# EnyaHermite/SPH3D-GCN

Hardware: AMD Instinct MI355X
Metric: point-cloud blocks/sec (fwd+bwd) SPH3D_s3dis 8192-pt (higher is better)
Workload: dtype f32

## Files before the change

### include/sph3d.h

```cpp
#ifndef SPH3D_H
#define SPH3D_H

#include <stddef.h>

#ifdef __cplusplus
extern "C" {
#endif

typedef void* sph3d_stream_t;

enum {
    SPH3D_OK = 0,
    SPH3D_EINVAL = -1,
    SPH3D_EWORKSPACE = -2,
    SPH3D_ELAUNCH = -3,
    SPH3D_EUNSUPPORTED = -4
};

#define SPH3D_ABI_VERSION 2
int sph3d_abi_version(void);
const char* sph3d_last_error(void);
const char* sph3d_build_info(void);


// ... 67 lines not shown
                                const int* nn_index, const int* nn_count, const int* bin_index,
                                const float* input, const float* filter, const float* grad_output,
                                float* grad_input, float* grad_filter,
                                void* workspace, size_t workspace_bytes,
                                sph3d_stream_t stream);

size_t sph3d_graph_transpose_workspace(int B, int N, int M, int K, int F);
int sph3d_graph_transpose(int B, int N, int M, int K, int F,
                          const int* nn_index, const int* nn_count,
                          const int* bin_index , const float* weight ,
                          int* offsets, int* ent_key, float* ent_scale,
                          int* active_bins ,
                          void* workspace, size_t workspace_bytes, sph3d_stream_t stream);
int sph3d_graph_transpose_count(int B, int N, int M, int K, int F, const int* nn_index, const int* nn_count,
                                const int* bin_index, int want_active, void* workspace, size_t workspace_bytes,
                                sph3d_stream_t stream);
int sph3d_graph_transpose_finish(int B, int N, int M, int K, int F,
                                 const int* nn_index, const int* nn_count, const int* bin_index,
                                 const float* weight, int* offsets, int* ent_key, float* ent_scale, int* active_bins,
                                 void* workspace, size_t workspace_bytes, sph3d_stream_t stream);
int sph3d_gather_rows_count(int B, int N, int S, int K, const int* pairs, const int* nn_index, const int* nn_count,
                            int* out_index, int* out_count, void* transpose_workspace, size_t transpose_workspace_bytes,
                            sph3d_stream_t stream);
int sph3d_graph_transpose_finish_ordered(int B, int N, int M, int K, int F,
                                         const int* nn_index, const int* nn_count, const int* bin_index,
                                         const float* weight, int* offsets, int* ent_key, float* ent_scale, int* active_bins,
                                         int* order, void* workspace, size_t workspace_bytes, sph3d_stream_t stream);
int sph3d_graph_balanced_order(int B, int N, int F, const int* offsets, int* order, sph3d_stream_t stream);
int sph3d_set_deterministic(int on);
int sph3d_get_deterministic(void);
size_t sph3d_graph_canonical_order_workspace(int B, int N, int M, int K, int F);
int sph3d_graph_canonical_order(int B, int N, int M, int K, int F, const int* offsets, int* ent_key, float* ent_scale ,
                                void* workspace, size_t workspace_bytes, sph3d_stream_t stream);
size_t sph3d_depthwise_conv3d_grad_t_workspace(int B, int N, int F, int C, int r);
int sph3d_depthwise_conv3d_grad_t(int B, int N, int M, int F, int C, int r,
                                  const int* offsets, const int* ent_key, const float* ent_scale,
                                  const int* source_order ,
                                  const int* active_bins ,
                                  const float* input, const float* filter, const float* grad_output,
                                  float* grad_input, float* grad_filter,
                                  void* workspace, size_t workspace_bytes, sph3d_stream_t stream);

int sph3d_fuzzy_spherical_kernel(int B, int N, int M, int K, int n, int p, int q, float radius,
                                 const float* database, const float* query,
                                 const int* nn_index, const int* nn_count, const float* nn_dist,
                                 int* filt_index, int* filt_frac, sph3d_stream_t stream);
// ... 6 lines not shown
                                      const int* offsets, const int* ent_edge,
                                      const float* input, const float* filter, const float* grad_output,
                                      float* grad_input, float* grad_filter,
                                      void* workspace, size_t workspace_bytes, sph3d_stream_t stream);
int sph3d_graph_transpose_finish_edges(int B, int N, int M, int K, const int* nn_index, const int* nn_count,
                                       int* offsets, int* ent_edge, void* workspace, size_t workspace_bytes,
                                       sph3d_stream_t stream);

int sph3d_scatter_grad_t(int B, int Nin, int Mout, int C,
                         const int* offsets, const int* ent_key, const float* ent_scale,
                         const float* grad_output, float* grad_input, sph3d_stream_t stream);
size_t sph3d_scatter_grad_workspace(int B, int N, int M, int K);

int sph3d_max_pool3d(int B, int N, int M, int C, int K,
                     const int* nn_index, const int* nn_count, const float* input,
                     float* output, int* max_index, sph3d_stream_t stream);
int sph3d_max_pool3d_grad(int B, int N, int M, int C,
                          const int* max_index, const float* grad_output,
                          float* grad_input, sph3d_stream_t stream);
int sph3d_max_pool3d_grad_t(int B, int N, int M, int C, const int* offsets, const int* ent_key, const int* nn_count,
                            const int* max_index, const float* grad_output,
                            const float* addend ,
                            float* grad_input, sph3d_stream_t stream);
int sph3d_avg_pool3d(int B, int N, int M, int C, int K,
                     const int* nn_index, const int* nn_count, const float* input,
                     float* output, sph3d_stream_t stream);
int sph3d_avg_pool3d_grad(int B, int N, int M, int C, int K,
                          const int* nn_index, const int* nn_count, const float* grad_output,
                          float* grad_input,
                          void* workspace , size_t workspace_bytes,
                          sph3d_stream_t stream);

int sph3d_mean_interpolate(int B, int N, int M, int C, int K,
                           const int* nn_index, const int* nn_count, const float* input,
                           float* output, sph3d_stream_t stream);
int sph3d_mean_interpolate_grad(int B, int N, int M, int C, int K,
                                const int* nn_index, const int* nn_count, const float* grad_output,
                                float* grad_input,
                                void* workspace , size_t workspace_bytes,
                                sph3d_stream_t stream);
int sph3d_weighted_interpolate(int B, int N, int M, int C, int K,
                               const int* nn_index, const int* nn_count,
                               const float* input, const float* weight,
                               float* output, sph3d_stream_t stream);
int sph3d_weighted_interpolate_grad(int B, int N, int M, int C, int K,
                                    const int* nn_index, const int* nn_count,
// ... 273 lines not shown
```

### sph3d_gcn_amd/_lib.py

```python
import ctypes
import os

import torch

_HERE = os.path.dirname(os.path.abspath(__file__))
LIB_PATH = os.environ.get("SPH3D_LIB") or os.path.join(_HERE, "csrc", "libsph3d.so")

_c_int = ctypes.c_int
_c_float = ctypes.c_float
_c_size_t = ctypes.c_size_t
_vp = ctypes.c_void_p

_I, _F, _P, _S, _L = _c_int, _c_float, _vp, _c_size_t, ctypes.c_longlong


class AugmentParams(ctypes.Structure):
    _fields_ = [("threshold", ctypes.c_ulonglong * 9), ("enable", ctypes.c_uint), ("rgb_offset", _I), ("normal_offset", _I),
                ("max_nodes", _I), ("rgb_lo", _F), ("rgb_hi", _F), ("inv_g", _F * 2), ("scale", _F * 2)]


SIGNATURES = {
    "sph3d_abi_version": (_I, []),
    "sph3d_last_error": (ctypes.c_char_p, []),
    "sph3d_build_info": (ctypes.c_char_p, []),
# ... 4 lines not shown
    "sph3d_build_sphere_neighbor_ws": (_I, [_I, _I, _I, _I, _F, _P, _P, _P, _P, _P, _P, _S, _P]),
    "sph3d_build_sphere_neighbor_fixed_ws": (_I, [_I, _I, _I, _I, _F, _P, _P, _P, _P, _P, _P, _S, _P]),
    "sph3d_release_stream_scratch": (_I, [_P]),
    "sph3d_release_all_scratch": (_I, []),
    "sph3d_build_sphere_graph_ws": (_I, [_I, _I, _I, _I, _F, _I, _I, _I, _I] + [_P] * 6 + [_P, _S, _P, _S, _P]),
    "sph3d_build_cube_neighbor": (_I, [_I, _I, _I, _I, _I, _F, _P, _P, _P, _P, _P]),
    "sph3d_spherical_kernel": (_I, [_I, _I, _I, _I, _I, _I, _I, _F, _P, _P, _P, _P, _P, _P, _P]),
    "sph3d_spherical_kernel_ocml": (_I, [_I, _I, _I, _I, _I, _I, _I, _F, _P, _P, _P, _P, _P, _P, _P]),
    "sph3d_depthwise_conv3d": (_I, [_I] * 7 + [_P] * 7),
    "sph3d_depthwise_conv3d_grad_workspace": (_S, [_I] * 7),
    "sph3d_depthwise_conv3d_grad": (_I, [_I] * 7 + [_P] * 8 + [_P, _S, _P]),
    "sph3d_max_pool3d": (_I, [_I] * 5 + [_P] * 6),
    "sph3d_max_pool3d_grad": (_I, [_I] * 4 + [_P] * 4),
    "sph3d_max_pool3d_grad_t": (_I, [_I] * 4 + [_P] * 8),
    "sph3d_avg_pool3d": (_I, [_I] * 5 + [_P] * 5),
    "sph3d_avg_pool3d_grad": (_I, [_I] * 5 + [_P] * 4 + [_P, _S, _P]),
    "sph3d_graph_balanced_order": (_I, [_I, _I, _I, _P, _P, _P]),
    "sph3d_set_deterministic": (_I, [_I]),
    "sph3d_get_deterministic": (_I, []),
    "sph3d_graph_canonical_order_workspace": (_S, [_I] * 5),
    "sph3d_graph_canonical_order": (_I, [_I] * 5 + [_P] * 3 + [_P, _S, _P]),
    "sph3d_gather_nd": (_I, [_I, _I, ctypes.c_longlong, _I, _P, _P, _P, _P]),
    "sph3d_gather_rows_count": (_I, [_I] * 4 + [_P] * 5 + [_P, _S, _P]),
    "sph3d_graph_transpose_workspace": (_S, [_I] * 5),
    "sph3d_graph_transpose": (_I, [_I] * 5 + [_P] * 8 + [_P, _S, _P]),
    "sph3d_graph_transpose_count": (_I, [_I] * 5 + [_P] * 3 + [_I, _P, _S, _P]),
    "sph3d_graph_transpose_finish": (_I, [_I] * 5 + [_P] * 8 + [_P, _S, _P]),
    "sph3d_graph_transpose_finish_ordered": (_I, [_I] * 5 + [_P] * 9 + [_P, _S, _P]),
    "sph3d_build_sphere_graph": (_I, [_I, _I, _I, _I, _F, _I, _I, _I] + [_P] * 6 + [_P, _S, _P]),
    "sph3d_build_sphere_graph_ocml": (_I, [_I, _I, _I, _I, _F, _I, _I, _I] + [_P] * 6 + [_P, _S, _P]),
    "sph3d_depthwise_conv3d_grad_t_workspace": (_S, [_I] * 5),
    "sph3d_depthwise_conv3d_grad_t": (_I, [_I] * 6 + [_P] * 10 + [_P, _S, _P]),
    "sph3d_fuzzy_spherical_kernel": (_I, [_I, _I, _I, _I, _I, _I, _I, _F] + [_P] * 7 + [_P]),
    "sph3d_fuzzy_depthwise_conv3d": (_I, [_I] * 10 + [_P] * 7 + [_P]),
    "sph3d_fuzzy_depthwise_conv3d_grad_workspace": (_S, [_I] * 7),
    "sph3d_fuzzy_depthwise_conv3d_grad": (_I, [_I] * 10 + [_P] * 11 + [_P, _S, _P]),
    "sph3d_graph_transpose_finish_edges": (_I, [_I] * 4 + [_P] * 4 + [_P, _S, _P]),
    "sph3d_depthwise_conv3d_cat_supported": (_I, [_I] * 4),
    "sph3d_depthwise_conv3d_cat": (_I, [_I] * 8 + [_P] * 8),
    "sph3d_depthwise_conv3d_grad_t_cat": (_I, [_I] * 7 + [_P] * 12 + [_P, _S, _P]),
    "sph3d_depthwise_conv3d_plan": (_I, [_I] * 11 + [_P]),
    "sph3d_spatial_order": (_I, [_I, _I, _P, _P, _P]),
    "sph3d_scatter_grad_t": (_I, [_I] * 4 + [_P] * 6),
    "sph3d_scatter_grad_workspace": (_S, [_I] * 4),
    "sph3d_mean_interpolate": (_I, [_I] * 5 + [_P] * 5),
    "sph3d_mean_interpolate_grad": (_I, [_I] * 5 + [_P] * 4 + [_P, _S, _P]),
# ... 121 lines not shown
            fn.restype = res
            fn.argtypes = args
    if l.sph3d_abi_version() != ABI_VERSION:
        raise Sph3dError("libsph3d.so ABI version %d, this package binds version %d" % (l.sph3d_abi_version(), ABI_VERSION))
    _lib = _Proxy(l)
    return _lib


_timing = None


def timing_start():
    global _timing
    _timing = []


def timing_stop():
    global _timing
    out, _timing = _timing, None
    return out


_PURE = ("_workspace", "_blocks", "_supported", "_parts", "_sample_chunk")
_NO_TIME = ("sph3d_abi_version", "sph3d_last_error", "sph3d_build_info", "workspace", "_release_", "_blocks", "_supported", "_launches", "_parts", "_failures", "_mode", "_pieces", "_sample_chunk", "_plan")


class _Proxy:

    def __init__(self, cdll):
        self._cdll = cdll
        self._cache = {}
        self._memos = []

    def __getattr__(self, name):
        fn = getattr(self._cdll, name)
        if name == "sph3d_set_deterministic":
            def switch(on, _fn=fn, _memos=self._memos):
                prev = _fn(on)
                if (prev != 0) != (on != 0):
                    for m in _memos:
                        m.clear()
                return prev
            self.__dict__[name] = switch
            return switch
        if any(k in name for k in _PURE) and name != "sph3d_pointwise_gemm_bnstats_blocks":
            memo = {}
            self._memos.append(memo)
# ... 154 lines not shown
```

### sph3d_gcn_amd/_tgraph.py

```python
import collections
import contextlib

import torch

from . import _lib

BALANCE_MIN_POINTS = 1024
PACK_ENTRIES = True
_MAX_ENTRIES = 24
_cache = collections.OrderedDict()


def _ident(t):
    return (0, 0) if t is None else (t.data_ptr(), t._version)


_generation = [0]


def clear():
    _lib.release_scratch()
    _cache.clear()
    _orders.clear()
    _unique.clear()
# ... 31 lines not shown


def source_order(nn_index):
    hit = _orders.get(_ident(nn_index))
    if hit is None:
        return None
    order = hit[0]
    if order.is_cuda:
        cur = _lib.current_raw_stream()
        if cur not in hit[2]:
            order.record_stream(torch.cuda.current_stream())
            hit[2].add(cur)
    return order


_unique = set()


def peek(nn_index, nn_count, n_src, need_unique_rows=False):
    key = (_ident(nn_index), _ident(nn_count), _ident(None), _ident(None), int(n_src), 1, tuple(nn_index.shape))
    if key not in _cache or (need_unique_rows and key not in _unique):
        return None
    return transpose(nn_index, nn_count, n_src)


def _attach(nn_index, fkey, hit, nn_count, bin_index, weight):
    fast = nn_index.__dict__.get("_sph3d_tg")
    if fast is None:
        fast = nn_index._sph3d_tg = {}
    out, _keep, ev, synced = hit
    fast[fkey] = ((out, (nn_count, bin_index, weight), ev, synced),
                  (_generation[0], nn_index._version, nn_count._version, 0 if bin_index is None else bin_index._version,
                   0 if weight is None else weight._version))


def entries(tg):
    _off, key, scale, _act = tg
    if scale is not None:
        return key, scale
    cnt = (key >> 24) & 0xff
    return key & 0xffffff, torch.where(cnt > 0, 1.0 / cnt.float().clamp(min=1.0), torch.zeros_like(cnt, dtype=torch.float32))


def transpose(nn_index, nn_count, n_src, bin_index=None, weight=None, num_bins=1, counted_workspace=None, unique_rows=False):
    F = int(num_bins) if bin_index is not None else 1
    cur_raw = _lib.current_raw_stream()
# ... 102 lines not shown
```

### sph3d_gcn_amd/csrc/common.hpp

```cpp
#pragma once
#include <hip/hip_runtime.h>
#include <stdint.h>
#include <stdio.h>
#include <stdlib.h>
#include "../../include/sph3d.h"

namespace sph3d {

constexpr int kWave = 64;
constexpr int kRefGrid = 32;
constexpr int kRefBlock = 1024;

void set_error(const char* fmt, ...);

#define SPH3D_REQUIRE(cond, ...)                    \
    do {                                            \
        if (!(cond)) {                              \
            ::sph3d::set_error(__VA_ARGS__);        \
            return SPH3D_EINVAL;                    \
        }                                           \
    } while (0)

static inline int check_launch(const char* what)
{
// ... 68 lines not shown
static inline TgLayout tg_layout(void* workspace, int B, int N, int M, int K, int F)
{
    size_t off = 0;
    auto take = [&](size_t bytes) {
        char* p = workspace ? (char*)workspace + off : nullptr;
        off += (bytes + 255) & ~(size_t)255;
        return p;
    };
    TgLayout t;
    t.offsets = (int*)take(sizeof(int) * (size_t)B * ((size_t)N * F + 1));
    t.key = (int*)take(sizeof(int) * (size_t)B * M * K);
    t.scale = (float*)take(sizeof(float) * (size_t)B * M * K);
    t.active = (int*)take(sizeof(int) * ((size_t)F + 1));
    const size_t scratch_off = off;
    t.scratch = take(sph3d_graph_transpose_workspace(B, N, M, K, F));
    t.scratch_bytes = off - scratch_off;
    t.bytes = off;
    return t;
}

constexpr unsigned kTgKeyMask = 0x00ffffffu;
static inline bool tg_packable(int M, int K, const void* weight) { return weight == nullptr && M <= (1 << 24) && K <= 255; }

constexpr int kVoteMaxClasses = 64;
static inline int vote_check_args(const char* what, int B, int C, int num_blocks, long long total_rows, long long row_base,
                                  long long batch_rows)
{
    SPH3D_REQUIRE(B > 0 && B <= 65535, "%s: batch 0<B<=65535 required, got %d", what, B);
    SPH3D_REQUIRE(C > 0 && C <= kVoteMaxClasses, "%s: 0<C<=%d classes required, got %d", what, kVoteMaxClasses, C);
    SPH3D_REQUIRE(num_blocks > 0 && total_rows > 0, "%s: empty pool (num_blocks=%d total_rows=%lld)", what, num_blocks, total_rows);
    SPH3D_REQUIRE(row_base >= 0 && batch_rows > 0 && batch_rows <= 0x7fffffffll && row_base + batch_rows <= total_rows,
                  "%s: rows [%lld, %lld + %lld) are not a range of the pool's %lld", what, row_base, row_base, batch_rows, total_rows);
    return SPH3D_OK;
}

__device__ __forceinline__ int lane_id() { return (int)(threadIdx.x & 63); }

__device__ __forceinline__ int tg_key(int word, bool packed) { return packed ? (int)((unsigned)word & kTgKeyMask) : word; }
__device__ __forceinline__ float tg_packed_scale(int word) { return 1.0f / (float)((unsigned)word >> 24); }

__device__ __forceinline__ int prefix_popc(unsigned long long mask)
{
    return (int)__builtin_amdgcn_mbcnt_hi((unsigned)(mask >> 32), __builtin_amdgcn_mbcnt_lo((unsigned)mask, 0u));
}

__device__ __forceinline__ float elu1(float y) { return y > 0.f ? y : __expf(y) - 1.f; }
// ... 70 lines not shown
```

### sph3d_gcn_amd/csrc/graph.hip

```cpp
#include "common.hpp"

namespace sph3d {

__global__ __launch_bounds__(256) void zero_fill_kernel(unsigned* __restrict__ p, size_t words)
{
    const size_t head = ((16 - (reinterpret_cast<size_t>(p) & 15)) & 15) >> 2;
    const size_t h = head < words ? head : words;
    uint4* q = reinterpret_cast<uint4*>(p + h);
    const size_t quads = (words - h) >> 2;
    const size_t stride = (size_t)gridDim.x * blockDim.x;
    const size_t t = (size_t)blockIdx.x * blockDim.x + threadIdx.x;
    for (size_t i = t; i < quads; i += stride) q[i] = make_uint4(0u, 0u, 0u, 0u);
    if (t < h) p[t] = 0u;
    const size_t tail0 = h + (quads << 2);
    if (t < words - tail0) p[tail0 + t] = 0u;
}

int zero_async(void* p, size_t bytes, hipStream_t stream, const char* what)
{
    if (bytes == 0) return SPH3D_OK;
    if (bytes < (256u << 10) || (bytes & 3) != 0 || (reinterpret_cast<size_t>(p) & 3) != 0)
        return check_hip(hipMemsetAsync(p, 0, bytes, stream), what);
    const size_t words = bytes >> 2;
    size_t blocks = (words / 4 + 255) / 256;
// ... 685 lines not shown
                                       sph3d_stream_t stream)
{
    SPH3D_REQUIRE(B > 0 && N > 0 && S >= 0 && K > 0, "gather_rows_count: bad dims B=%d N=%d S=%d K=%d", B, N, S, K);
    if (S == 0) return SPH3D_OK;
    hipStream_t st = as_stream(stream);
    int* deg = nullptr;
    int* slot = nullptr;
    if (transpose_workspace != nullptr) {
        int rc = tg_dims_ok(B, N, S, K, 1, nullptr, transpose_workspace, transpose_workspace_bytes);
        if (rc) return rc;
        const TgWs w = tg_ws(transpose_workspace, B, N, S, K, 1);
        rc = zero_async(w.deg, sizeof(int) * w.zero_words, st, "gather_rows_count: memset");
        if (rc) return rc;
        deg = w.deg;
        slot = w.slot_pos;
    }
    long long blocks = ((long long)B * S + 3) / 4;
    if (blocks > 16384) blocks = 16384;
    hipLaunchKernelGGL(gather_rows_count_kernel, dim3((unsigned)blocks), dim3(256), 0, st, B, N, S, K, pairs, nn_index, nn_count, out_index,
                       out_count, deg, slot);
    return check_launch("sph3d_gather_rows_count");
}

extern "C" int sph3d_graph_transpose(int B, int N, int M, int K, int F,
                                     const int* nn_index, const int* nn_count, const int* bin_index,
                                     const float* weight, int* offsets, int* ent_key, float* ent_scale, int* active_bins,
                                     void* workspace, size_t workspace_bytes, sph3d_stream_t stream)
{
    int rc = sph3d_graph_transpose_count(B, N, M, K, F, nn_index, nn_count, bin_index, active_bins != nullptr, workspace,
                                         workspace_bytes, stream);
    if (rc) return rc;
    return sph3d_graph_transpose_finish(B, N, M, K, F, nn_index, nn_count, bin_index, weight, offsets, ent_key, ent_scale,
                                        active_bins, workspace, workspace_bytes, stream);
}
```

### sph3d_gcn_amd/csrc/pool3d.hip

```cpp
#include "common.hpp"

namespace sph3d {

constexpr int kPtsPerWG = 16;

enum class Mode { Max, Avg, Weighted };

template <Mode MODE, int V>
__global__ __launch_bounds__(256) void gather_fwd(
    int B, int Nin, int Mout, int C, int K, int mblocks,
    const int* __restrict__ nnIndex, const int* __restrict__ nnCount,
    const float* __restrict__ input, const float* __restrict__ weight,
    float* __restrict__ output, int* __restrict__ maxIndex, int ppwg)
{
    int b, mb;
    xcd_decode((int)blockIdx.x, B, mblocks, b, mb);
    if (b < 0) return;
    const int wave = uniform((int)threadIdx.x >> 6);
    const int lane = lane_id();
    const int m_begin = mb * ppwg;
    const int m_end = (m_begin + ppwg) < Mout ? (m_begin + ppwg) : Mout;
    const float* inb = input + (size_t)b * Nin * C;

    for (int m = m_begin + wave; m < m_end; m += 4) {
// ... 214 lines not shown
    for (int n = n_begin + wave; n < n_end; n += 4) {
        const int e0 = offb[n], e1 = offb[n + 1];
        for (int c0 = 0; c0 < C; c0 += 64 * V) {
            const int c = c0 + lane * V;
            const bool act = c < C;
            const int cc = act ? c : 0;
            float acc[V];
#pragma unroll
            for (int v = 0; v < V; v++) acc[v] = addend != nullptr ? addend[((size_t)b * Nin + n) * C + cc + v] : 0.f;
            auto take = [&](int m) {
                if (V == 4) {
                    const int4 a = *reinterpret_cast<const int4*>(&mib[(size_t)m * C + cc]);
                    const float4 g = *reinterpret_cast<const float4*>(&gob[(size_t)m * C + cc]);
                    acc[0] += a.x == n ? g.x : 0.f;
                    acc[1 % V] += a.y == n ? g.y : 0.f;
                    acc[2 % V] += a.z == n ? g.z : 0.f;
                    acc[3 % V] += a.w == n ? g.w : 0.f;
                } else {
                    acc[0] += mib[(size_t)m * C + cc] == n ? gob[(size_t)m * C + cc] : 0.f;
                }
            };
#pragma unroll 4
            for (int e = e0; e < e1; e++) take(Mout <= (1 << 24) ? (int)((unsigned)entKey[e] & kTgKeyMask) : entKey[e]);
            if (n == 0) {
                for (int m0 = 0; m0 < Mout; m0 += 64) {
                    const int mm = m0 + lane;
                    const int cnt = mm < Mout ? nnCount[(size_t)b * Mout + mm] : 1;
                    unsigned long long empty = __ballot(cnt == 0);
                    while (empty != 0ull) {
                        const int bit = (int)__builtin_ctzll(empty);
                        empty &= empty - 1ull;
                        take(m0 + bit);
                    }
                }
            }
            if (act) {
#pragma unroll
                for (int v = 0; v < V; v++) gradInput[((size_t)b * Nin + n) * C + c + v] = acc[v];
            }
        }
    }
}

template <int V>
__global__ __launch_bounds__(256) void gather_bwd_t_split(
    int B, int Nin, int Mout, int C,
// ... 237 lines not shown
    hipLaunchKernelGGL(maxpool_bwd, dim3((unsigned)blocks, (unsigned)B), dim3(256), 0, st, B, N, M, C, max_index, grad_output, grad_input);
    return check_launch("sph3d_max_pool3d_grad");
}

extern "C" int sph3d_max_pool3d_grad_t(int B, int N, int M, int C, const int* offsets, const int* ent_key, const int* nn_count,
                                       const int* max_index, const float* grad_output, const float* addend, float* grad_input,
                                       sph3d_stream_t stream)
{
    SPH3D_REQUIRE(B >= 0 && N > 0 && M >= 0 && C > 0, "MaxPool3dGrad: bad dims B=%d N=%d M=%d C=%d", B, N, M, C);
    if (B == 0) return SPH3D_OK;
    hipStream_t st = as_stream(stream);
    const int ppwg = (long long)B * N >= 65536 ? kPtsPerWG : 4;
    const int nblocks = (N + ppwg - 1) / ppwg;
    const dim3 grid(xcd_grid(B, nblocks));
    if (C % 4 == 0)
        hipLaunchKernelGGL(maxpool_bwd_t<4>, grid, dim3(256), 0, st, B, N, M, C, nblocks, ppwg, offsets, ent_key, nn_count, max_index,
                           grad_output, addend, grad_input);
    else
        hipLaunchKernelGGL(maxpool_bwd_t<1>, grid, dim3(256), 0, st, B, N, M, C, nblocks, ppwg, offsets, ent_key, nn_count, max_index,
                           grad_output, addend, grad_input);
    return check_launch("sph3d_max_pool3d_grad_t");
}

extern "C" int sph3d_avg_pool3d(int B, int N, int M, int C, int K, const int* nn_index, const int* nn_count,
                                const float* input, float* output, sph3d_stream_t stream)
{
    return launch_fwd<Mode::Avg>("sph3d_avg_pool3d", B, N, M, C, K, nn_index, nn_count, input, nullptr, output,
                                 nullptr, as_stream(stream));
}



extern "C" int sph3d_scatter_grad_t(int B, int Nin, int Mout, int C, const int* offsets, const int* ent_key,
                                    const float* ent_scale, const float* grad_output, float* grad_input,
                                    sph3d_stream_t stream)
{
    return launch_bwd_t("sph3d_scatter_grad_t", B, Nin, Mout, C, offsets, ent_key, ent_scale, grad_output, grad_input,
                        as_stream(stream));
}

extern "C" size_t sph3d_scatter_grad_workspace(int B, int N, int M, int K) { return tg_layout(nullptr, B, N, M, K, 1).bytes; }

static int grad_via_transpose(const char* who, int B, int Nin, int Mout, int C, int K, const int* nn_index,
                              const int* nn_count, const float* weight, const float* grad_output, float* grad_input,
                              void* workspace, size_t workspace_bytes, sph3d_stream_t stream)
{
// ... 97 lines not shown
```

### sph3d_gcn_amd/harness/s3dis_net.py

```python
import copy
import types

import torch
import torch.nn.functional as F

from .. import _lib
from .. import sph3gcn_util as s3g_util


def s3dis_config(num_input=8192):
    c = types.SimpleNamespace()
    c.num_input = num_input
    c.num_cls = 13
    c.mlp = 64
    c.num_sample = [2048, 768, 384, 128]
    c.radius = [0.1, 0.2, 0.4, 0.8]
    c.nn_uplimit = [64, 64, 64, 64]
    c.channels = [[128, 128], [256, 256], [256, 256], [512, 512]]
    c.multiplier = [[2, 2], [2, 2], [2, 2], [2, 2]]
    c.weight_decay = None
    c.kernel = [8, 2, 2]
    c.binSize = 8 * 2 * 2 + 1
    c.normalize = True
    c.pool_method = 'max'
# ... 174 lines not shown
            self.events.append(ev)

    def _intra_graph(self, xyz, radius, uplimit):
        c = self.config
        if self._fuzzy:
            idx, cnt, dst = s3g_util.neighbor_fn(xyz, xyz, radius=radius, nnsample=uplimit)
            return idx, cnt, dst, s3g_util.fuzzy_spherical_kernel(xyz, xyz, idx, cnt, dst, radius, kernel=c.kernel)
        return s3g_util.build_intra_graph(xyz, radius, uplimit, c.kernel, **self._bw_kw())

    def _make_enc(self, l):
        c = self.config
        xyz = self.xyz_layers[l]
        idx, cnt, dst, filt = self._intra_graph(xyz, c.radius[l], c.nn_uplimit[l])
        if self._ids:
            return dict(intra_idx=idx, intra_cnt=cnt, filt_idx=filt, intra_dst=dst)
        return dict(intra_idx=idx, intra_cnt=cnt, filt_idx=filt)

    def _bw_kw(self):
        return {} if self.need_backward else {"with_transpose": False}

    def _make_pool(self, l, g):
        fused = getattr(s3g_util, "gather_pooling_graph", None)
        if fused is not None and g["intra_idx"].is_cuda:
            g["inter_idx"], g["inter_cnt"] = fused(g["intra_idx"], g["intra_cnt"], self.indices[l],
                                                   with_transpose=self.config.pool_method == 'max' and self.need_backward)
            return
        g["inter_idx"] = s3g_util.gather_nd(g["intra_idx"], self.indices[l])
        g["inter_cnt"] = s3g_util.gather_nd(g["intra_cnt"], self.indices[l])
        if self.config.pool_method == 'max' and g["inter_idx"].is_cuda and self.need_backward:
            from .. import _tgraph
            _tgraph.transpose(g["inter_idx"], g["inter_cnt"], self.xyz_layers[l].shape[1], unique_rows=True)

    def _make_dec(self, l):
        c = self.config
        L = len(c.radius)
        radius, uplimit = c.radius[L - 1 - l], c.nn_uplimit[L - 1 - l]
        xyz_c, xyz_unpool = self.xyz_layers[L - l], self.xyz_layers[L - 1 - l]
        intra_idx, intra_cnt, intra_dst, filt_idx = self._intra_graph(xyz_c, radius, uplimit)
        from .. import tf_nnquery
        unpool_k = getattr(c, "unpool_k", None)
        if unpool_k is not None:
            inter_idx, inter_cnt, inter_dst = tf_nnquery.build_nearest_neighbor(xyz_c, xyz_unpool, unpool_k, dist="squared")
        elif (self.need_backward and xyz_c.is_cuda and c.unpool_method == 'mean' and s3g_util.neighbor_fn is s3g_util.build_sphere_neighbor
                and tf_nnquery.get_radius_mode() == "compat"):
            inter_idx, inter_cnt, inter_dst = tf_nnquery.build_sphere_neighbor_counted(xyz_c, xyz_unpool, radius, uplimit)
        else:
# ... 236 lines not shown
```

### sph3d_gcn_amd/sph3gcn_util.py

```python
import contextlib
import math

import torch
import torch.nn.functional as F

from . import tf_conv3d, tf_pool3d, tf_unpool3d
from .tf_nnquery import build_sphere_neighbor, build_cube_neighbor
from .tf_sample import farthest_point_sample, inverse_density_sample, inverse_density_sample_keyed, random_sample
from .tf_buildkernel import spherical_kernel, fuzzy_spherical_kernel
from . import tf_gemm, tf_norm, _lib

neighbor_fn = build_sphere_neighbor

elu = F.elu


class VariableStore(torch.nn.Module):

    def __init__(self, device=None, seed=None):
        super().__init__()
        self.params = torch.nn.ParameterDict()
        self._device = device
        self._gen = None
        if seed is not None:
# ... 188 lines not shown
    return params[b, p]


def gather_pooling_graph(nn_index, nn_count, indices, with_transpose=True):
    if not (nn_index.is_cuda and nn_index.dim() == 3 and nn_count.dim() == 2 and indices.dtype == torch.int32 and indices.shape[-1] == 2
            and indices.shape[0] == nn_index.shape[0]):
        return gather_nd(nn_index, indices), gather_nd(nn_count, indices)
    from . import _tgraph
    nn_index, nn_count, indices = nn_index.contiguous(), nn_count.contiguous(), indices.contiguous()
    B, N, K = nn_index.shape
    S = indices.shape[1]
    dev = nn_index.device
    out_idx = _lib.empty((B, S, K), torch.int32, dev)
    out_cnt = _lib.empty((B, S), torch.int32, dev)
    l = _lib.lib()
    ws, wsb = None, 0
    if with_transpose:
        wsb = l.sph3d_graph_transpose_workspace(B, N, S, K, 1)
        ws = torch.empty((max(wsb, 1),), dtype=torch.uint8, device=dev)
    _lib.check(l.sph3d_gather_rows_count(B, N, S, K, _lib.ptr(indices), _lib.ptr(nn_index), _lib.ptr(nn_count), _lib.ptr(out_idx),
                                         _lib.ptr(out_cnt), _lib.ptr(ws), wsb, _lib.stream_ptr()))
    if with_transpose:
        _tgraph.transpose(out_idx, out_cnt, N, counted_workspace=ws, unique_rows=True)
    return out_idx, out_cnt


def _finish(outputs, num_out_channels, scope, activation_fn, with_bn, with_bias, reuse, is_training, fused_bias=None):
    if with_bias and fused_bias is None:
        biases = get_variable_store().get_variable(scope + '/biases', [num_out_channels], _constant(0.0))
        outputs = outputs + biases
    if (with_bn and activation_fn is elu and FUSE_ELU_BN and outputs.is_cuda and tf_norm.supported(outputs.shape[-1])):
        return _elu_batch_normalization(outputs, is_training, name=scope + '/bn')
    if activation_fn is not None:
        outputs = activation_fn(outputs)
    if with_bn:
        outputs = batch_normalization(outputs, is_training, name=scope + '/bn', reuse=reuse)
    return outputs


def _fused_tail_applies(x2d, num_out_channels, activation_fn, with_bn, with_bias, is_training):
    training = True if is_training is None else bool(is_training)
    return (FUSE_GEMM_BN and FUSE_ELU_BN and with_bn and activation_fn is elu and training and x2d.is_cuda
            and tf_norm.supported(num_out_channels)
            and tf_norm.gemm_bn_blocks(x2d.shape[0], x2d.shape[1], num_out_channels) > 0)


# ... 351 lines not shown
```

### sph3d_gcn_amd/tf_pool3d.py

```python
from typing import Tuple

import torch

from . import _lib, _tgraph


def _check_pool(input, nn_index, nn_count):
    if input.dim() != 3:
        raise ValueError("rank of input should be 3")
    if nn_index.dim() != 3:
        raise ValueError("rank of nn_index should be 3")
    if nn_count.dim() != 2:
        raise ValueError("rank of nn_count should be 2")


def _max_pool3d_impl(input: torch.Tensor, nn_index: torch.Tensor, nn_count: torch.Tensor) -> Tuple[torch.Tensor, torch.Tensor]:
    _lib.require_device(input, nn_index, nn_count)
    _check_pool(input, nn_index, nn_count)
    input, nn_index, nn_count = _lib.f32(input), _lib.i32(nn_index), _lib.i32(nn_count)
    B, N, C = input.shape
    M, K = nn_index.shape[1], nn_index.shape[2]
    output = torch.empty((B, M, C), dtype=torch.float32, device=input.device)
    max_index = torch.empty((B, M, C), dtype=torch.int32, device=input.device)
    _lib.check(_lib.lib().sph3d_max_pool3d(B, N, M, C, K, _lib.ptr(nn_index), _lib.ptr(nn_count), _lib.ptr(input),
# ... 87 lines not shown
    ctx.save_for_backward(*inputs)


def _avg_backward(ctx, grad_output):
    input, nn_index, nn_count = ctx.saved_tensors
    return _avg_pool3d_grad(input, grad_output, nn_index, nn_count), None, None


_avg_pool3d.register_autograd(_avg_backward, setup_context=_avg_setup)


def _max_pool3d_grad_t_impl(input, grad_output, max_index, nn_count, tg, addend=None):
    grad_output, max_index = _lib.f32(grad_output), _lib.i32(max_index)
    addend = None if addend is None else _lib.f32(addend)
    B, N, C = input.shape
    M = grad_output.shape[1]
    grad_input = torch.empty((B, N, C), dtype=torch.float32, device=input.device)
    _lib.check(_lib.lib().sph3d_max_pool3d_grad_t(B, N, M, C, _lib.ptr(tg[0]), _lib.ptr(tg[1]), _lib.ptr(nn_count),
                                                  _lib.ptr(max_index), _lib.ptr(grad_output), _lib.ptr(addend), _lib.ptr(grad_input),
                                                  _lib.stream_ptr()))
    return grad_input


def _no_scatter_when_deterministic():
    if _tgraph.is_deterministic():
        raise RuntimeError("max_pool3d backward: deterministic mode is on and no transposed pooling graph with unique rows is cached for "
                           "this (nn_index, nn_count); the scatter form adds with float atomics.  Build the pooling graph with "
                           "unique_rows=True (sph3gcn_util.gather_pooling_graph, or _tgraph.transpose(nn_index, nn_count, N, "
                           "unique_rows=True)) while the mode is on")


class _MaxPool3dFn(torch.autograd.Function):
    @staticmethod
    def forward(ctx, input, nn_index, nn_count):
        output, max_index = _max_pool3d_impl(input, nn_index, nn_count)
        ctx.save_for_backward(input, max_index, nn_index, nn_count)
        ctx.mark_non_differentiable(max_index)
        return output, max_index

    @staticmethod
    def backward(ctx, grad_output, grad_index):
        input, max_index, nn_index, nn_count = ctx.saved_tensors
        tg = None
        if input.is_cuda and nn_index.dtype == torch.int32 and nn_count.dtype == torch.int32:
            tg = _tgraph.peek(nn_index, nn_count, input.shape[1], need_unique_rows=True)
        if tg is not None:
            return _max_pool3d_grad_t_impl(input, grad_output, max_index, nn_count, tg), None, None
        _no_scatter_when_deterministic()
        return _max_pool3d_grad_impl(input, grad_output, max_index), None, None


class _AvgPool3dFn(torch.autograd.Function):
    @staticmethod
    def forward(ctx, input, nn_index, nn_count):
        ctx.save_for_backward(input, nn_index, nn_count)
        return _avg_pool3d_impl(input, nn_index, nn_count)

    @staticmethod
    def backward(ctx, grad_output):
        input, nn_index, nn_count = ctx.saved_tensors
        return _avg_pool3d_grad_impl(input, grad_output, nn_index, nn_count), None, None


def max_pool3d(input, nn_index, nn_count):
    return _MaxPool3dFn.apply(input, nn_index, nn_count)


class _MaxPool3dSkipFn(torch.autograd.Function):

    @staticmethod
    def forward(ctx, input, nn_index, nn_count):
        output, max_index = _max_pool3d_impl(input, nn_index, nn_count)
        ctx.save_for_backward(input, max_index, nn_index, nn_count)
        ctx.mark_non_differentiable(max_index)
        return output, max_index, input.view_as(input)

    @staticmethod
    def backward(ctx, grad_output, grad_index, grad_skip):
        input, max_index, nn_index, nn_count = ctx.saved_tensors
        tg = None
        if input.is_cuda and nn_index.dtype == torch.int32 and nn_count.dtype == torch.int32:
            tg = _tgraph.peek(nn_index, nn_count, input.shape[1], need_unique_rows=True)
        if grad_output is None:
            return grad_skip, None, None
        if tg is not None:
            skip = grad_skip.contiguous() if grad_skip is not None else None
            return _max_pool3d_grad_t_impl(input, grad_output, max_index, nn_count, tg, addend=skip), None, None
        _no_scatter_when_deterministic()
        g = _max_pool3d_grad_impl(input, grad_output, max_index)
        return (g if grad_skip is None else g + grad_skip), None, None


def max_pool3d_with_skip(input, nn_index, nn_count):
    return _MaxPool3dSkipFn.apply(input, nn_index, nn_count)


def max_pool3d_grad(input, grad_output, max_index):
    return _max_pool3d_grad_impl(input, grad_output, max_index)


def avg_pool3d(input, nn_index, nn_count):
    return _AvgPool3dFn.apply(input, nn_index, nn_count)


def avg_pool3d_grad(input, grad_output, nn_index, nn_count):
    return _avg_pool3d_grad_impl(input, grad_output, nn_index, nn_count)
```

Baseline: 2174.

## Reuse intra-graph transpose with row linked lists for max-pool backward

Builds the pooling graph with a new gather kernel that also records, for each source point, a linked list of the pooled rows that copied it (first/next arrays built with atomics). Max-pool backward then reuses the already-cached transposed intra-level graph, walking each source's linked rows, instead of building a separate unique-row transpose of the pooling graph. This removes the extra transpose build in the forward setup. In exchange the backward kernel does more indirect, divergent chain walking, the row order is nondeterministic, and the path is disabled in deterministic mode.

```diff
diff --git a/include/sph3d.h b/include/sph3d.h
--- a/include/sph3d.h
+++ b/include/sph3d.h
@@ -113,6 +113,8 @@
 int sph3d_gather_rows_count(int B, int N, int S, int K, const int* pairs, const int* nn_index, const int* nn_count,
                             int* out_index, int* out_count, void* transpose_workspace, size_t transpose_workspace_bytes,
                             sph3d_stream_t stream);
+int sph3d_gather_rows_link(int B, int N, int S, int K, const int* pairs, const int* nn_index, const int* nn_count,
+                           int* out_index, int* out_count, int* first, int* next, sph3d_stream_t stream);
 int sph3d_graph_transpose_finish_ordered(int B, int N, int M, int K, int F,
                                          const int* nn_index, const int* nn_count, const int* bin_index,
                                          const float* weight, int* offsets, int* ent_key, float* ent_scale, int* active_bins,
@@ -165,6 +167,9 @@
                             const int* max_index, const float* grad_output,
                             const float* addend ,
                             float* grad_input, sph3d_stream_t stream);
+int sph3d_max_pool3d_grad_rows(int B, int N, int M, int C, int F, const int* offsets, const int* ent_key, const int* first,
+                               const int* next, const int* nn_count, const int* max_index, const float* grad_output,
+                               const float* addend , float* grad_input, sph3d_stream_t stream);
 int sph3d_avg_pool3d(int B, int N, int M, int C, int K,
                      const int* nn_index, const int* nn_count, const float* input,
                      float* output, sph3d_stream_t stream);
diff --git a/sph3d_gcn_amd/_lib.py b/sph3d_gcn_amd/_lib.py
--- a/sph3d_gcn_amd/_lib.py
+++ b/sph3d_gcn_amd/_lib.py
@@ -50,6 +50,8 @@
     "sph3d_graph_canonical_order": (_I, [_I] * 5 + [_P] * 3 + [_P, _S, _P]),
     "sph3d_gather_nd": (_I, [_I, _I, ctypes.c_longlong, _I, _P, _P, _P, _P]),
     "sph3d_gather_rows_count": (_I, [_I] * 4 + [_P] * 5 + [_P, _S, _P]),
+    "sph3d_gather_rows_link": (_I, [_I] * 4 + [_P] * 7 + [_P]),
+    "sph3d_max_pool3d_grad_rows": (_I, [_I] * 5 + [_P] * 10),
     "sph3d_graph_transpose_workspace": (_S, [_I] * 5),
     "sph3d_graph_transpose": (_I, [_I] * 5 + [_P] * 8 + [_P, _S, _P]),
     "sph3d_graph_transpose_count": (_I, [_I] * 5 + [_P] * 3 + [_I, _P, _S, _P]),
@@ -217,7 +219,7 @@
 
 
 _PURE = ("_workspace", "_blocks", "_supported", "_parts", "_sample_chunk")
-_NO_TIME = ("sph3d_abi_version", "sph3d_last_error", "sph3d_build_info", "workspace", "_release_", "_blocks", "_supported", "_launches", "_parts", "_failures", "_mode", "_pieces", "_sample_chunk", "_plan")
+_NO_TIME = ("sph3d_abi_version", "sph3d_last_error", "sph3d_build_info", "sph3d_get_deterministic", "workspace", "_release_", "_blocks", "_supported", "_launches", "_parts", "_failures", "_mode", "_pieces", "_sample_chunk", "_plan")
 
 
 class _Proxy:
diff --git a/sph3d_gcn_amd/_tgraph.py b/sph3d_gcn_amd/_tgraph.py
--- a/sph3d_gcn_amd/_tgraph.py
+++ b/sph3d_gcn_amd/_tgraph.py
@@ -77,6 +77,39 @@
     if key not in _cache or (need_unique_rows and key not in _unique):
         return None
     return transpose(nn_index, nn_count, n_src)
+
+
+def cached(nn_index, nn_count, n_src, bin_index=None, num_bins=1):
+    F = int(num_bins) if bin_index is not None else 1
+    key = (_ident(nn_index), _ident(nn_count), _ident(bin_index), _ident(None), int(n_src), F, tuple(nn_index.shape))
+    if key not in _cache:
+        return None
+    return transpose(nn_index, nn_count, n_src, bin_index=bin_index, num_bins=num_bins)
+
+
+def attach_row_link(pool_index, pool_count, first, next_, intra_index, intra_count, bin_index, num_bins):
+    ev = torch.cuda.Event()
+    ev.record(torch.cuda.current_stream())
+    pool_index._sph3d_rows = ((first, next_, intra_index, intra_count, bin_index, int(num_bins), ev, {_lib.current_raw_stream()}),
+                              pool_count, (_generation[0], pool_index._version, pool_count._version))
+
+
+def row_link(pool_index, pool_count):
+    hung = pool_index.__dict__.get("_sph3d_rows")
+    if hung is None or hung[1] is not pool_count or hung[2] != (_generation[0], pool_index._version, pool_count._version):
+        return None
+    first, next_, intra_index, intra_count, bin_index, num_bins, ev, synced = hung[0]
+    tg = cached(intra_index, intra_count, intra_index.shape[1], bin_index=bin_index, num_bins=num_bins)
+    if tg is None:
+        return None
+    cur_raw = _lib.current_raw_stream()
+    if cur_raw not in synced:
+        cur = torch.cuda.current_stream()
+        cur.wait_event(ev)
+        first.record_stream(cur)
+        next_.record_stream(cur)
+        synced.add(cur_raw)
+    return first, next_, tg, (num_bins if bin_index is not None else 1)
 
 
 def _attach(nn_index, fkey, hit, nn_count, bin_index, weight):
diff --git a/sph3d_gcn_amd/csrc/common.hpp b/sph3d_gcn_amd/csrc/common.hpp
--- a/sph3d_gcn_amd/csrc/common.hpp
+++ b/sph3d_gcn_amd/csrc/common.hpp
@@ -114,6 +114,9 @@
 constexpr unsigned kTgKeyMask = 0x00ffffffu;
 static inline bool tg_packable(int M, int K, const void* weight) { return weight == nullptr && M <= (1 << 24) && K <= 255; }
 
+constexpr unsigned kRowLinkMore = 0x80000000u;
+constexpr unsigned kRowLinkMask = 0x7fffffffu;
+
 constexpr int kVoteMaxClasses = 64;
 static inline int vote_check_args(const char* what, int B, int C, int num_blocks, long long total_rows, long long row_base,
                                   long long batch_rows)
diff --git a/sph3d_gcn_amd/csrc/graph.hip b/sph3d_gcn_amd/csrc/graph.hip
--- a/sph3d_gcn_amd/csrc/graph.hip
+++ b/sph3d_gcn_amd/csrc/graph.hip
@@ -731,6 +731,51 @@
     return check_launch("sph3d_gather_rows_count");
 }
 
+__global__ __launch_bounds__(256) void gather_rows_link_kernel(int B, int N, int S, int K, const int* __restrict__ pairs,
+                                                               const int* __restrict__ nnIndex, const int* __restrict__ nnCount,
+                                                               int* __restrict__ outIndex, int* __restrict__ outCount,
+                                                               int* __restrict__ first, int* __restrict__ next)
+{
+    const int lane = (int)threadIdx.x & 63;
+    const long long rows = (long long)B * S;
+    for (long long s = (long long)blockIdx.x * 4 + ((int)threadIdx.x >> 6); s < rows; s += (long long)gridDim.x * 4) {
+        int b = pairs[s * 2], p = pairs[s * 2 + 1];
+        b = b < 0 ? 0 : (b >= B ? B - 1 : b);
+        p = p < 0 ? 0 : (p >= N ? N - 1 : p);
+        const int ob = (int)(s / S);
+        const long long src = ((long long)b * N + p);
+        if (lane == 0) {
+            outCount[s] = nnCount[src];
+            int* head = &first[(size_t)ob * N + p];
+            const int old = atomicExch(head, (int)(s - (long long)ob * S) + 1);
+            next[s] = (int)((unsigned)old & kRowLinkMask);
+            if (old != 0) atomicOr(head, (int)kRowLinkMore);
+        }
+        for (int k = lane; k < K; k += 64) outIndex[s * K + k] = nnIndex[src * K + k];
+    }
+}
+
+extern "C" int sph3d_gather_rows_link(int B, int N, int S, int K, const int* pairs, const int* nn_index, const int* nn_count,
+                                      int* out_index, int* out_count, int* first, int* next, sph3d_stream_t stream)
+{
+    SPH3D_REQUIRE(B > 0 && N > 0 && S >= 0 && K > 0, "gather_rows_link: bad dims B=%d N=%d S=%d K=%d", B, N, S, K);
+    SPH3D_REQUIRE((unsigned)S < kRowLinkMore - 1u, "gather_rows_link: S=%d rows per cloud do not fit the link word", S);
+    SPH3D_REQUIRE(first != nullptr && (next != nullptr || S == 0), "gather_rows_link: first [B, N] and next [B, S] are required");
+    if (deterministic_on()) {
+        set_error("gather_rows_link: deterministic mode is on and a chain of rows that copy one point is linked in arrival order; use "
+                  "sph3d_gather_rows_count and the pooling graph's own transposed graph");
+        return SPH3D_EUNSUPPORTED;
+    }
+    hipStream_t st = as_stream(stream);
+    int rc = zero_async(first, sizeof(int) * (size_t)B * N, st, "gather_rows_link: memset");
+    if (rc || S == 0) return rc;
+    long long blocks = ((long long)B * S + 3) / 4;
+    if (blocks > 16384) blocks = 16384;
+    hipLaunchKernelGGL(gather_rows_link_kernel, dim3((unsigned)blocks), dim3(256), 0, st, B, N, S, K, pairs, nn_index, nn_count, out_index,
+                       out_count, first, next);
+    return check_launch("sph3d_gather_rows_link");
+}
+
 extern "C" int sph3d_graph_transpose(int B, int N, int M, int K, int F,
                                      const int* nn_index, const int* nn_count, const int* bin_index,
                                      const float* weight, int* offsets, int* ent_key, float* ent_scale, int* active_bins,
diff --git a/sph3d_gcn_amd/csrc/pool3d.hip b/sph3d_gcn_amd/csrc/pool3d.hip
--- a/sph3d_gcn_amd/csrc/pool3d.hip
+++ b/sph3d_gcn_amd/csrc/pool3d.hip
@@ -260,6 +260,96 @@
             };
 #pragma unroll 4
             for (int e = e0; e < e1; e++) take(Mout <= (1 << 24) ? (int)((unsigned)entKey[e] & kTgKeyMask) : entKey[e]);
+            if (n == 0) {
+                for (int m0 = 0; m0 < Mout; m0 += 64) {
+                    const int mm = m0 + lane;
+                    const int cnt = mm < Mout ? nnCount[(size_t)b * Mout + mm] : 1;
+                    unsigned long long empty = __ballot(cnt == 0);
+                    while (empty != 0ull) {
+                        const int bit = (int)__builtin_ctzll(empty);
+                        empty &= empty - 1ull;
+                        take(m0 + bit);
+                    }
+                }
+            }
+            if (act) {
+#pragma unroll
+                for (int v = 0; v < V; v++) gradInput[((size_t)b * Nin + n) * C + c + v] = acc[v];
+            }
+        }
+    }
+}
+
+template <int V>
+__global__ __launch_bounds__(256) void maxpool_bwd_rows(
+    int B, int Nin, int Mout, int C, int F, int nblocks, int ppwg,
+    const int* __restrict__ offsets, const int* __restrict__ entKey, const int* __restrict__ first, const int* __restrict__ next,
+    const int* __restrict__ nnCount, const int* __restrict__ maxIndex, const float* __restrict__ gradOutput,
+    const float* __restrict__ addend, float* __restrict__ gradInput)
+{
+    int b, nb;
+    xcd_decode((int)blockIdx.x, B, nblocks, b, nb);
+    if (b < 0) return;
+    const int wave = uniform((int)threadIdx.x >> 6);
+    const int lane = lane_id();
+    const int n_begin = nb * ppwg;
+    const int n_end = (n_begin + ppwg) < Nin ? (n_begin + ppwg) : Nin;
+    const float* gob = gradOutput + (size_t)b * Mout * C;
+    const int* mib = maxIndex + (size_t)b * Mout * C;
+    const int* __restrict__ offb = offsets + (size_t)b * ((size_t)Nin * F + 1);
+    const int* __restrict__ firstb = first + (size_t)b * Nin;
+    const int* __restrict__ nextb = next + (size_t)b * Mout;
+    for (int n = n_begin + wave; n < n_end; n += 4) {
+        const int e0 = offb[(size_t)n * F], e1 = offb[(size_t)n * F + F];
+        for (int c0 = 0; c0 < C; c0 += 64 * V) {
+            const int c = c0 + lane * V;
+            const bool act = c < C;
+            const int cc = act ? c : 0;
+            float acc[V];
+#pragma unroll
+            for (int v = 0; v < V; v++) acc[v] = addend != nullptr ? addend[((size_t)b * Nin + n) * C + cc + v] : 0.f;
+            auto take = [&](int m) {
+                if (V == 4) {
+                    const int4 a = *reinterpret_cast<const int4*>(&mib[(size_t)m * C + cc]);
+                    const float4 g = *reinterpret_cast<const float4*>(&gob[(size_t)m * C + cc]);
+                    acc[0] += a.x == n ? g.x : 0.f;
+                    acc[1 % V] += a.y == n ? g.y : 0.f;
+                    acc[2 % V] += a.z == n ? g.z : 0.f;
+                    acc[3 % V] += a.w == n ? g.w : 0.f;
+                } else {
+                    acc[0] += mib[(size_t)m * C + cc] == n ? gob[(size_t)m * C + cc] : 0.f;
+                }
+            };
+            for (int ec = e0; ec < e1; ec += 64) {
+                const int e = ec + lane;
+                int link = 0;
+                if (e < e1) link = firstb[Nin <= (1 << 24) ? (int)((unsigned)entKey[e] & kTgKeyMask) : entKey[e]];
+                const unsigned long long hit = __ballot(link != 0);
+                if (hit == 0ull) continue;
+                const int hits = (int)__popcll(hit);
+                const int below = prefix_popc(hit);
+                const int rows = __builtin_amdgcn_ds_permute((link != 0 ? below : hits + lane - below) << 2, link);
+                auto row = [&](int i) { return (int)((unsigned)__builtin_amdgcn_readlane(rows, i) & kRowLinkMask) - 1; };
+                int i = 0;
+                for (; i + 4 <= hits; i += 4) {
+                    const int r0 = row(i), r1 = row(i + 1), r2 = row(i + 2), r3 = row(i + 3);
+                    take(r0);
+                    take(r1);
+                    take(r2);
+                    take(r3);
+                }
+                for (; i < hits; i++) take(row(i));
+                unsigned long long more = __ballot(link < 0);
+                while (more != 0ull) {
+                    const int bit = (int)__builtin_ctzll(more);
+                    more &= more - 1ull;
+                    int r = nextb[(int)((unsigned)__builtin_amdgcn_readlane(link, bit) & kRowLinkMask) - 1];
+                    while (r != 0) {
+                        take(r - 1);
+                        r = nextb[r - 1];
+                    }
+                }
+            }
             if (n == 0) {
                 for (int m0 = 0; m0 < Mout; m0 += 64) {
                     const int mm = m0 + lane;
@@ -543,6 +633,26 @@
     return check_launch("sph3d_max_pool3d_grad_t");
 }
 
+extern "C" int sph3d_max_pool3d_grad_rows(int B, int N, int M, int C, int F, const int* offsets, const int* ent_key, const int* first,
+                                          const int* next, const int* nn_count, const int* max_index, const float* grad_output,
+                                          const float* addend, float* grad_input, sph3d_stream_t stream)
+{
+    SPH3D_REQUIRE(B >= 0 && N > 0 && M >= 0 && C > 0 && F > 0, "MaxPool3dGrad: bad dims B=%d N=%d M=%d C=%d F=%d", B, N, M, C, F);
+    SPH3D_REQUIRE((long long)N * F < 0x7fffffffll, "MaxPool3dGrad: N=%d sources of F=%d segments exceed the offsets' index range", N, F);
+    if (B == 0) return SPH3D_OK;
+    hipStream_t st = as_stream(stream);
+    const int ppwg = (long long)B * N >= 65536 ? kPtsPerWG : 4;
+    const int nblocks = (N + ppwg - 1) / ppwg;
+    const dim3 grid(xcd_grid(B, nblocks));
+    if (C % 4 == 0)
+        hipLaunchKernelGGL(maxpool_bwd_rows<4>, grid, dim3(256), 0, st, B, N, M, C, F, nblocks, ppwg, offsets, ent_key, first, next, nn_count,
+                           max_index, grad_output, addend, grad_input);
+    else
+        hipLaunchKernelGGL(maxpool_bwd_rows<1>, grid, dim3(256), 0, st, B, N, M, C, F, nblocks, ppwg, offsets, ent_key, first, next, nn_count,
+                           max_index, grad_output, addend, grad_input);
+    return check_launch("sph3d_max_pool3d_grad_rows");
+}
+
 extern "C" int sph3d_avg_pool3d(int B, int N, int M, int C, int K, const int* nn_index, const int* nn_count,
                                 const float* input, float* output, sph3d_stream_t stream)
 {
diff --git a/sph3d_gcn_amd/harness/s3dis_net.py b/sph3d_gcn_amd/harness/s3dis_net.py
--- a/sph3d_gcn_amd/harness/s3dis_net.py
+++ b/sph3d_gcn_amd/harness/s3dis_net.py
@@ -220,6 +220,14 @@
     def _make_pool(self, l, g):
         fused = getattr(s3g_util, "gather_pooling_graph", None)
         if fused is not None and g["intra_idx"].is_cuda:
+            from .. import _tgraph
+            if (self.config.pool_method == 'max' and self.need_backward and not self._fuzzy and not _tgraph.is_deterministic()
+                    and hasattr(s3g_util, "gather_pooling_rows")
+                    and _tgraph.cached(g["intra_idx"], g["intra_cnt"], g["intra_idx"].shape[1], bin_index=g["filt_idx"],
+                                       num_bins=self.config.binSize) is not None):
+                g["inter_idx"], g["inter_cnt"] = s3g_util.gather_pooling_rows(g["intra_idx"], g["intra_cnt"], self.indices[l],
+                                                                              bin_index=g["filt_idx"], num_bins=self.config.binSize)
+                return
             g["inter_idx"], g["inter_cnt"] = fused(g["intra_idx"], g["intra_cnt"], self.indices[l],
                                                    with_transpose=self.config.pool_method == 'max' and self.need_backward)
             return
diff --git a/sph3d_gcn_amd/sph3gcn_util.py b/sph3d_gcn_amd/sph3gcn_util.py
--- a/sph3d_gcn_amd/sph3gcn_util.py
+++ b/sph3d_gcn_amd/sph3gcn_util.py
@@ -234,6 +234,23 @@
                                          _lib.ptr(out_cnt), _lib.ptr(ws), wsb, _lib.stream_ptr()))
     if with_transpose:
         _tgraph.transpose(out_idx, out_cnt, N, counted_workspace=ws, unique_rows=True)
+    return out_idx, out_cnt
+
+
+def gather_pooling_rows(nn_index, nn_count, indices, bin_index=None, num_bins=1):
+    from . import _tgraph
+    nn_index, nn_count, indices = nn_index.contiguous(), nn_count.contiguous(), indices.contiguous()
+    B, N, K = nn_index.shape
+    S = indices.shape[1]
+    dev = nn_index.device
+    out_idx = _lib.empty((B, S, K), torch.int32, dev)
+    out_cnt = _lib.empty((B, S), torch.int32, dev)
+    first = _lib.empty((B, N), torch.int32, dev)
+    nxt = _lib.empty((B, S), torch.int32, dev)
+    _lib.check(_lib.lib().sph3d_gather_rows_link(B, N, S, K, _lib.ptr(indices), _lib.ptr(nn_index), _lib.ptr(nn_count),
+                                                 _lib.ptr(out_idx), _lib.ptr(out_cnt), _lib.ptr(first), _lib.ptr(nxt),
+                                                 _lib.stream_ptr()))
+    _tgraph.attach_row_link(out_idx, out_cnt, first, nxt, nn_index, nn_count, bin_index, num_bins)
     return out_idx, out_cnt
 
 
diff --git a/sph3d_gcn_amd/tf_pool3d.py b/sph3d_gcn_amd/tf_pool3d.py
--- a/sph3d_gcn_amd/tf_pool3d.py
+++ b/sph3d_gcn_amd/tf_pool3d.py
@@ -133,6 +133,31 @@
     return grad_input
 
 
+def _max_pool3d_grad_rows_impl(input, grad_output, max_index, nn_count, link, addend=None):
+    first, nxt, tg, F = link
+    grad_output, max_index = _lib.f32(grad_output), _lib.i32(max_index)
+    addend = None if addend is None else _lib.f32(addend)
+    B, N, C = input.shape
+    M = grad_output.shape[1]
+    grad_input = torch.empty((B, N, C), dtype=torch.float32, device=input.device)
+    _lib.check(_lib.lib().sph3d_max_pool3d_grad_rows(B, N, M, C, F, _lib.ptr(tg[0]), _lib.ptr(tg[1]), _lib.ptr(first), _lib.ptr(nxt),
+                                                     _lib.ptr(nn_count), _lib.ptr(max_index), _lib.ptr(grad_output), _lib.ptr(addend),
+                                                     _lib.ptr(grad_input), _lib.stream_ptr()))
+    return grad_input
+
+
+def _gather_form(input, nn_index, nn_count):
+    if not (input.is_cuda and nn_index.dtype == torch.int32 and nn_count.dtype == torch.int32):
+        return None
+    tg = _tgraph.peek(nn_index, nn_count, input.shape[1], need_unique_rows=True)
+    if tg is not None:
+        return "t", tg
+    link = _tgraph.row_link(nn_index, nn_count)
+    if link is None or tuple(link[0].shape) != tuple(input.shape[:2]):
+        return None
+    return "rows", link
+
+
 def _no_scatter_when_deterministic():
     if _tgraph.is_deterministic():
         raise RuntimeError("max_pool3d backward: deterministic mode is on and no transposed pooling graph with unique rows is cached for "
@@ -152,11 +177,10 @@
     @staticmethod
     def backward(ctx, grad_output, grad_index):
         input, max_index, nn_index, nn_count = ctx.saved_tensors
-        tg = None
-        if input.is_cuda and nn_index.dtype == torch.int32 and nn_count.dtype == torch.int32:
-            tg = _tgraph.peek(nn_index, nn_count, input.shape[1], need_unique_rows=True)
-        if tg is not None:
-            return _max_pool3d_grad_t_impl(input, grad_output, max_index, nn_count, tg), None, None
+        form = _gather_form(input, nn_index, nn_count)
+        if form is not None:
+            impl = _max_pool3d_grad_t_impl if form[0] == "t" else _max_pool3d_grad_rows_impl
+            return impl(input, grad_output, max_index, nn_count, form[1]), None, None
         _no_scatter_when_deterministic()
         return _max_pool3d_grad_impl(input, grad_output, max_index), None, None
 
@@ -189,14 +213,13 @@
     @staticmethod
     def backward(ctx, grad_output, grad_index, grad_skip):
         input, max_index, nn_index, nn_count = ctx.saved_tensors
-        tg = None
-        if input.is_cuda and nn_index.dtype == torch.int32 and nn_count.dtype == torch.int32:
-            tg = _tgraph.peek(nn_index, nn_count, input.shape[1], need_unique_rows=True)
         if grad_output is None:
             return grad_skip, None, None
-        if tg is not None:
+        form = _gather_form(input, nn_index, nn_count)
+        if form is not None:
             skip = grad_skip.contiguous() if grad_skip is not None else None
-            return _max_pool3d_grad_t_impl(input, grad_output, max_index, nn_count, tg, addend=skip), None, None
+            impl = _max_pool3d_grad_t_impl if form[0] == "t" else _max_pool3d_grad_rows_impl
+            return impl(input, grad_output, max_index, nn_count, form[1], addend=skip), None, None
         _no_scatter_when_deterministic()
         g = _max_pool3d_grad_impl(input, grad_output, max_index)
         return (g if grad_skip is None else g + grad_skip), None, None
```

Measured after the change: 2200 (median of 6 runs). 1.2% higher.
